# loxxous/Jampack

Measured on AMD Instinct MI355X. Metric: MB/s compress (forward BWT + rANS encode) on 64 MiB blocks; bit-exact vs CPU ref, higher is better.
Workload: dtype u8/int32; 1 GPU; enwik8-like 100000000 B per GPU as 64 MiB blocks (2 blocks), forward BWT + rANS encode, inputs resident in HBM

## Files before the change

### jampack_amd/csrc/ans_enc.hip

```cpp
#include <vector>

#include "ans_enc.hpp"
#include "chain_pool.hpp"

using namespace jpk;
using namespace jpk_enc;

namespace {

void enc_layout(Arena &a, const EncDims &d, EncBufs &b, int what, size_t sym_total = 0, size_t lane_total = 0)
{
    const size_t tiles = (size_t)d.nch * d.tpc;
    const size_t stride = d.chunk;
    const size_t nsym = sym_total ? sym_total : (size_t)d.nch * stride;
    const size_t nlane = lane_total ? lane_total : (size_t)d.nch * 4 * rans_lane_stride(stride);
    const EncBufs keep = b;
    if (what & LAY_RANK) memset(&b, 0, sizeof b); else b = keep;
    if (what & LAY_RANK) {
        b.tilecnt = a.get<uint32_t>(tiles * 256);
        b.lastpos = a.get<int32_t>(tiles * 256);
        b.freq = a.get<int32_t>((size_t)d.nch * 256);
        b.bstart = a.get<uint32_t>((size_t)d.nch * 256);
        b.ranks = a.get<uint8_t>((size_t)d.nch * stride + 64);
    }
    if (what & LAY_RLE) {
        b.lz = a.get<uint32_t>(tiles);
        b.ext = a.get<uint32_t>(tiles);
        b.tcount = a.get<uint32_t>(tiles);
        b.toff = a.get<uint32_t>(tiles);
        b.rlen = a.get<uint32_t>(d.nch + 1);
        b.rle = a.get<uint16_t>((size_t)d.nch * stride + 64);
    }
    if (what & LAY_MODEL) {
        b.dens = a.get<uint32_t>(d.nch + 64);
        b.cmap = a.get<uint32_t>(d.nch + 64);
        b.clscnt = a.get<uint32_t>(tiles * 8);
        b.clstotal = a.get<uint32_t>((size_t)d.nch * 8);
        b.ord = a.get<uint32_t>(nsym);
        b.qhist = a.get<uint32_t>((size_t)d.nch * 6 * NQ * QSTRIDE);
        b.qcdf = a.get<uint32_t>((size_t)d.nch * 6 * NQ * QSTRIDE);
        b.exph = a.get<uint16_t>(7 * nsym);
        b.mantad = a.get<uint32_t>(nsym);
        b.cls8 = a.get<uint8_t>(nsym + 64);
        b.clist = a.get<uint32_t>(2 * ((nsym + 3) & ~(size_t)3) + 64);
        const size_t segs = (size_t)d.nch * 9 * d.tpc;
        b.seg_flag = a.get<uint32_t>(segs);
        b.seg_lo = a.get<int32_t>(segs);
        b.seg_end = a.get<int32_t>(segs);
        b.seg_start = a.get<int32_t>(segs);
        b.seg_tab = a.get<uint16_t>(segs * 32);
        b.seg_miss = a.get<uint16_t>(segs);
        b.seg_reach = a.get<uint16_t>(segs);
        b.recs = a.get<uint4>(nlane + RANS_SLACK) + (a.planning ? 0 : RANS_SLACK);
        b.pairs = (what & LAY_PLAIN) ? a.get<uint32_t>((size_t)d.nch * stride * 2) : nullptr;
    }
    if (what & LAY_RANS) {
        b.x16 = a.get<uint16_t>(nlane + 64);
        b.emask = a.get<uint32_t>(nlane / 16 + 64);
        b.etsum = a.get<uint32_t>((size_t)d.nch * emit_tiles_per_chunk(stride));
        b.fstate = a.get<uint32_t>((size_t)d.nch * 4);
        b.csize = a.get<uint32_t>(d.nch);
        b.stamp = a.get<uint64_t>(2 * (size_t)d.nch);
        b.hdr = a.get<uint8_t>((size_t)d.nch * HDR_MAX);
        b.hsize = a.get<uint32_t>(d.nch);
// ... 109 lines not shown
        Arena rest(ctx, true);
        EncBufs dummy = b;
        enc_layout(rest, d, dummy, LAY_MODEL | LAY_RANS, sym_total ? sym_total : 256, lane_total ? lane_total : 512);
        if (ctx->arena_off + rest.need > ctx->arena_cap) {
            if (attempt) return JPK_E_ALLOC;
            JPK_TRY(jpk_arena_ensure(ctx, ctx->arena_off + rest.need));
            continue;
        }
        enc_layout(real, d, b, LAY_MODEL | LAY_RANS, sym_total ? sym_total : 256, lane_total ? lane_total : 512);
        d.sbase = sbase; d.lbase = lbase;
        break;
    }
    return JPK_OK;
}

int enc_launch_groups(jpk_ctx *ctx, int inflight_n, uint32_t nch)
{
    int ngroups = jpk_enc_groups_for(inflight_n, nch);
    static const long groups_env = jpk_env_long("JPK_ENC_GROUPS", 0);
    if (groups_env >= 1 && groups_env <= jpk_ctx::ENC_GROUPS && (uint32_t)groups_env <= nch) ngroups = groups_env;
    for (int g = 0; g + 1 < ngroups; g++)
        if (!ctx->aux[g] && hipStreamCreateWithFlags(&ctx->aux[g], hipStreamNonBlocking) != hipSuccess) { ctx->aux[g] = nullptr; ngroups = g + 1; break; }
    return ngroups;
}

int enc_graded_groups(jpk_ctx *ctx, const uint8_t *d_in, const EncDims &d, EncBufs &b, int ngroups)
{
    hipStream_t st = ctx->stream;
    JPK_HIP(hipMemsetAsync(b.dens, 0, (size_t)d.nch * 4, st));
    JPK_LAUNCH(ctx, PROF_ENC_HIST, d.len, k_density, dim3((d.chunk + ATILE * 4 - 1) / (ATILE * 4), d.nch), dim3(TB), d_in, d, b.dens);
    JPK_LAUNCH(ctx, PROF_ENC_HIST, 0, k_order, dim3(1), dim3(256), d, b.dens, b.cmap);
    JPK_HIP(hipEventRecord(ctx->ev_pre[0], st));
    uint32_t gsz[jpk_ctx::ENC_GROUPS];
    {
        uint32_t left = d.nch;
        for (int g = 0; g < ngroups; g++) {
            uint32_t n = (g + 1 == ngroups) ? left : d.nch >> (ngroups - g);
            if (n < 2) n = 2;
            if (n > left) n = left;
            gsz[g] = n;
            left -= n;
        }
    }
    uint32_t off = 0;
// ... 38 lines not shown
        JPK_TRY(rc);
        JPK_HIP(hipGetLastError());
        JPK_HIP(hipEventRecord(ctx->ev_done[0], lease.stream));
        JPK_HIP(hipEventSynchronize(ctx->ev_done[0]));
        lease.done();
    } else {
        JPK_TRY(run_chain(ctx, d, b));
    }
    JPK_TRY(run_emit_counts(ctx, d, b));
    return JPK_OK;
}

int encode_core(jpk_ctx *ctx, const uint8_t *d_in, EncDims &d, EncBufs &b, int inflight_n, const GroupTabs *gt = nullptr)
{
    JPK_TRY(enc_front(ctx, d_in, d, b, gt));
    JPK_HIP(hipMemsetAsync(b.qhist, 0, (size_t)d.nch * 6 * NQ * QSTRIDE * 4, ctx->stream));
    const int ngroups = enc_launch_groups(ctx, inflight_n, d.nch);
    if (ngroups >= 2) JPK_TRY(enc_graded_groups(ctx, d_in, d, b, ngroups));
    else JPK_TRY(enc_single_group(ctx, d, b));
    return run_offsets(ctx, d, b);
}
}

size_t jpk_ans_encode_arena_bytes(uint32_t len)
{
    if (len == 0) return 0;
    const EncDims d = make_dims(len, ANS_CHUNK);
    return enc_plan_bytes(d, 0, ENC_PLAN_SYM_256);
}
size_t jpk_ans_encode_arena_bytes_worst(uint32_t len)
{
// ... 130 lines not shown
}

int jpk_model_pairs_device(jpk_ctx *ctx, const uint16_t *d_rle, int32_t rlen, uint32_t *d_pairs)
{
    if (rlen == 0) return JPK_OK;
    const EncDims d = make_dims((uint32_t)rlen, (uint32_t)rlen);
    EncBufs b;
    Arena plan(ctx, true);
    enc_layout(plan, d, b, LAY_RLE | LAY_MODEL | LAY_PLAIN);
    JPK_TRY(jpk_arena_ensure(ctx, plan.need));
    Arena real(ctx, false);
    enc_layout(real, d, b, LAY_RLE | LAY_MODEL | LAY_PLAIN);
    uint32_t n = (uint32_t)rlen;
    JPK_HIP(hipMemcpyAsync(b.rlen, &n, 4, hipMemcpyHostToDevice, ctx->stream));
    JPK_HIP(hipStreamSynchronize(ctx->stream));
    JPK_HIP(hipMemsetAsync(b.qhist, 0, (size_t)d.nch * 6 * NQ * QSTRIDE * 4, ctx->stream));
    JPK_TRY(run_model(ctx, d_rle, b.rlen, d, b));
    JPK_TRY(run_pairs(ctx, d_rle, b.rlen, d, b));
    JPK_HIP(hipMemcpyAsync(d_pairs, b.pairs, (size_t)rlen * 8, hipMemcpyDeviceToDevice, ctx->stream));
    JPK_HIP(hipStreamSynchronize(ctx->stream));
    return JPK_OK;
}
```

### jampack_amd/csrc/ans_enc.hpp

```cpp
#pragma once
#include "ans_common.hpp"
#include "common.hpp"

namespace jpk_enc {
using namespace jpk;

constexpr int TB = 256;

struct EncDims {
    uint32_t len;
    uint32_t chunk;
    uint32_t nch;
    uint32_t tpc;
    uint32_t ncl;
    const uint32_t *cmap;
    const uint32_t *clen;
    const uint32_t *cblk;
    uint8_t *const *bout;
    const uint32_t *sbase;
    const uint32_t *lbase;
};
__device__ __forceinline__ uint32_t chunk_of(const EncDims &d, uint32_t i) { return d.cmap ? d.cmap[i] : i; }
__device__ __forceinline__ size_t sym_stride(const EncDims &d, uint32_t c, size_t rle_stride) { return d.sbase ? (size_t)(d.sbase[c + 1] - d.sbase[c]) : rle_stride; }
__device__ __forceinline__ size_t sym_base(const EncDims &d, uint32_t c, size_t rle_stride) { return d.sbase ? (size_t)d.sbase[c] : (size_t)c * rle_stride; }
// ... 5 lines not shown
    return left < d.chunk ? (uint32_t)left : d.chunk;
}

__host__ __device__ __forceinline__ size_t rans_lane_stride(size_t rle_stride) { return (rle_stride / 2 + 384) & ~(size_t)127; }
__device__ __forceinline__ size_t lane_stride_of(const EncDims &d, uint32_t c, size_t rle_stride) { return rans_lane_stride(sym_stride(d, c, rle_stride)); }
__device__ __forceinline__ size_t lane_base(const EncDims &d, uint32_t c, size_t rle_stride) { return d.lbase ? (size_t)d.lbase[c] : (size_t)c * 4 * rans_lane_stride(rle_stride); }

constexpr int RANS_RING = 16;
constexpr int RANS_SLACK = 16 * RANS_RING;
constexpr int ETILE = 4096;
constexpr int HDR_MAX = 259 * 5 + 1;
inline uint32_t emit_tiles_per_chunk(size_t stride) { return (uint32_t)((2 * stride + ETILE - 1) / ETILE); }

struct EncBufs {
    uint32_t *tilecnt; int32_t *lastpos; int32_t *freq; uint32_t *bstart; uint8_t *ranks;
    uint32_t *lz, *ext, *tcount, *toff, *rlen;
    uint16_t *rle;
    uint32_t *clscnt, *clstotal, *ord, *qhist, *qcdf, *dens, *cmap;
    uint8_t *cls8; uint32_t *clist;
    uint32_t *seg_flag; int32_t *seg_lo, *seg_end, *seg_start; uint16_t *seg_tab, *seg_miss, *seg_reach;
    uint16_t *exph; uint32_t *mantad, *pairs; uint4 *recs;
    uint16_t *x16; uint32_t *emask, *etsum, *fstate, *csize;
    uint64_t *stamp;
    uint8_t *hdr; uint32_t *hsize; uint64_t *outoff;
};

enum { LAY_RANK = 1, LAY_RLE = 2, LAY_MODEL = 4, LAY_RANS = 8, LAY_PLAIN = 16 };

constexpr int MAIL_TOTAL = 0;
constexpr int MAIL_RLE_SYMBOLS = 2;
constexpr int MAIL_CHAIN_CYCLES = 4;
constexpr int MAIL_CHAIN_TICKS = 6;
constexpr int MAIL_CHAIN_RLEN = 8;
constexpr int MAIL_SYM_TOTAL = 12;
constexpr int MAIL_LANE_TOTAL = 13;
// ... 20 lines not shown
```

### jampack_amd/csrc/ans_enc_front.hip

```cpp
#include "ans_enc.hpp"

using namespace jpk;
using namespace jpk_enc;

namespace {

__global__ __launch_bounds__(TB) void k_enc_hist(const uint8_t *__restrict__ in, EncDims d, uint32_t *__restrict__ tilecnt,
                                                int32_t *__restrict__ lastpos)
{
    const uint32_t c = chunk_of(d, blockIdx.y), t = blockIdx.x;
    const uint32_t clen = chunk_len(d, c), ts = t * ATILE;
    if (ts >= clen) return;
    __shared__ uint32_t h[TB / 64][256];
    __shared__ int32_t lp[TB / 64][256];
#pragma unroll
    for (int k = 0; k < TB / 64; k++) { h[k][threadIdx.x] = 0; lp[k][threadIdx.x] = -1; }
    __syncthreads();
    const uint8_t *src = in + (size_t)c * d.chunk;
    uint8_t sy[ATILE / TB];
#pragma unroll
    for (int it = 0; it < ATILE / TB; it++) {
        const uint32_t i = ts + it * TB + threadIdx.x;
        sy[it] = src[i < clen ? i : clen - 1];
    }
// ... 8 lines not shown
        if (valid && (m & lt) == 0ull) {
            h[w][s] += (uint32_t)__popcll(m);
            lp[w][s] = (int32_t)(i - (uint32_t)lane_id() + (63u - (uint32_t)__clzll((long long)m)));
        }
    }
    __syncthreads();
    size_t o = ((size_t)c * d.tpc + t) * 256 + threadIdx.x;
    uint32_t hs = 0;
    int32_t lm = -1;
#pragma unroll
    for (int k = 0; k < TB / 64; k++) { hs += h[k][threadIdx.x]; lm = lp[k][threadIdx.x] > lm ? lp[k][threadIdx.x] : lm; }
    tilecnt[o] = hs;
    lastpos[o] = lm;
}

__global__ __launch_bounds__(256) void k_enc_prep(EncDims d, uint32_t *__restrict__ tilecnt, int32_t *__restrict__ lastpos,
                                                 int32_t *__restrict__ freq, uint32_t *__restrict__ bstart)
{
    const uint32_t c = chunk_of(d, blockIdx.x), s = threadIdx.x;
    const uint32_t clen = chunk_len(d, c);
    const uint32_t nt = (clen + ATILE - 1) / ATILE;
    uint32_t f = 0;
    int32_t p = -1;
    for (uint32_t t = 0; t < nt; t++) {
        size_t o = ((size_t)c * d.tpc + t) * 256 + s;
        uint32_t n = tilecnt[o];
        tilecnt[o] = f;
        f += n;
        int32_t l = lastpos[o];
        lastpos[o] = p;
        p = l > p ? l : p;
    }
    __shared__ uint32_t sf[256];
    sf[s] = f;
    freq[(size_t)c * 256 + s] = (int32_t)f;
    __syncthreads();
    uint32_t b = 0;
    for (uint32_t k = 0; k < 256; k++) {
        uint32_t fk = sf[k];
        if (fk > f || (fk == f && k < s)) b += fk;
    }
    bstart[(size_t)c * 256 + s] = b;
}

__device__ __forceinline__ uint32_t mtf_shr1(uint32_t carry_in, uint32_t v)
{
// ... 127 lines not shown
    for (int k = 0; k < ATILE / TB; k++) {
        const uint32_t p = k * TB + threadIdx.x;
        rv[k] = src[p < tl ? p : tl - 1];
    }
#pragma unroll
    for (int k = ATILE / TB - 1; k >= 0; k--) {
        uint32_t p = k * TB + threadIdx.x;
        if (p < tl && rv[k] != 0) first = p;
    }
    __shared__ uint32_t sm[TB / 64 + 1];
    uint32_t tot;
    block_incl_scan<OpMin>(first, sm, &tot);
    if (threadIdx.x == 0) lz[(size_t)c * d.tpc + t] = tot < tl ? tot : tl;
}

__global__ void k_rle_ext(EncDims d, const uint32_t *__restrict__ lz, uint32_t *__restrict__ ext)
{
    const uint32_t ci = blockIdx.x * blockDim.x + threadIdx.x;
    if (ci >= d.ncl) return;
    const uint32_t c = chunk_of(d, ci);
    const uint32_t clen = chunk_len(d, c);
    const uint32_t nt = (clen + ATILE - 1) / ATILE;
    uint32_t e = 0;
    for (int t = (int)nt - 1; t >= 0; t--) {
        ext[(size_t)c * d.tpc + t] = e;
        uint32_t tl = (clen - t * ATILE < (uint32_t)ATILE) ? clen - t * ATILE : (uint32_t)ATILE;
        uint32_t z = lz[(size_t)c * d.tpc + t];
        e = (z == tl) ? z + e : z;
    }
}

template <bool EMIT>
__global__ __launch_bounds__(TB) void k_rle_tiles(const uint8_t *__restrict__ ranks, EncDims d, const uint32_t *__restrict__ ext,
                                                 uint32_t *__restrict__ tcount, const uint32_t *__restrict__ toff, uint16_t *__restrict__ rle,
                                                 size_t rle_stride)
{
    const uint32_t c = chunk_of(d, blockIdx.y), t = blockIdx.x;
    const uint32_t clen = chunk_len(d, c), ts = t * ATILE;
    if (ts >= clen) return;
    const uint32_t tl = (clen - ts < (uint32_t)ATILE) ? clen - ts : (uint32_t)ATILE;
    const uint8_t *src = ranks + (size_t)c * d.chunk + ts;
    const uint32_t p0 = threadIdx.x * 16;
    uint8_t v[16];
#pragma unroll
    for (int k = 0; k < 16; k++) v[k] = (p0 + k < tl) ? src[p0 + k] : (uint8_t)1;
    uint32_t first = 0xFFFFFFFFu;
#pragma unroll
    for (int k = 15; k >= 0; k--)
        if (p0 + k < tl && v[k] != 0) first = p0 + k;
    __shared__ uint32_t fz[TB];
    __shared__ uint32_t res[TB];
    __shared__ uint32_t sm[TB / 64 + 1];
    fz[threadIdx.x] = first;
    __syncthreads();
    uint32_t rv = fz[TB - 1 - threadIdx.x];
    uint32_t inc = block_incl_scan<OpMin>(rv, sm, nullptr);
    res[threadIdx.x] = inc;
    __syncthreads();
    uint32_t after = (threadIdx.x == TB - 1) ? 0xFFFFFFFFu : res[TB - 2 - threadIdx.x];
    if (after == 0xFFFFFFFFu) after = tl + ext[(size_t)c * d.tpc + t];
    uint32_t nxt[16];
    uint32_t nn = after;
#pragma unroll
    for (int k = 15; k >= 0; k--) {
        nxt[k] = nn;
        if (p0 + k < tl && v[k] != 0) nn = p0 + k;
    }
    uint32_t prev;
    if (p0 == 0) prev = (ts == 0) ? 1u : src[-1];
    else prev = (p0 - 1 < tl) ? src[p0 - 1] : 1u;
    uint32_t cnt = 0;
    uint32_t pv = prev;
#pragma unroll
    for (int k = 0; k < 16; k++) {
        if (p0 + k < tl) {
            if (v[k] != 0) cnt += 1;
            else if (pv != 0) {
                uint32_t L = nxt[k] - (p0 + k) + 1;
                cnt += 31 - __clz((int)L);
            }
            pv = v[k];
        }
    }
    uint32_t tot;
    uint32_t incl = block_incl_scan<OpSum>(cnt, sm, &tot);
    if (!EMIT) {
        if (threadIdx.x == 0) tcount[(size_t)c * d.tpc + t] = tot;
        return;
    }
    uint16_t *out = rle + (size_t)c * rle_stride + toff[(size_t)c * d.tpc + t] + (incl - cnt);
    pv = prev;
#pragma unroll
    for (int k = 0; k < 16; k++) {
        if (p0 + k < tl) {
            if (v[k] != 0) *out++ = (uint16_t)(v[k] + 1);
            else if (pv != 0) {
                uint32_t L = nxt[k] - (p0 + k) + 1;
                for (int b = 30 - __clz((int)L); b >= 0; b--) *out++ = (uint16_t)((L >> b) & 1u);
            }
            pv = v[k];
        }
    }
}

__global__ void k_tile_prefix(EncDims d, const uint32_t *__restrict__ tcount, uint32_t *__restrict__ toff, uint32_t *__restrict__ total,
                              uint32_t unit_from_len , const uint32_t *__restrict__ count_in)
{
    const uint32_t ci = blockIdx.x * blockDim.x + threadIdx.x;
    if (ci >= d.ncl) return;
    const uint32_t c = chunk_of(d, ci);
    const uint32_t n = unit_from_len ? chunk_len(d, c) : count_in[c];
    const uint32_t nt = (n + ATILE - 1) / ATILE;
    uint32_t s = 0;
    for (uint32_t t = 0; t < nt; t++) {
        uint32_t v = tcount[(size_t)c * d.tpc + t];
        toff[(size_t)c * d.tpc + t] = s;
        s += v;
    }
    total[c] = s;
}

}

namespace jpk_enc {

int run_rank(jpk_ctx *ctx, const uint8_t *d_in, const EncDims &d, EncBufs &b)
{
    JPK_LAUNCH(ctx, PROF_ENC_HIST, d.len, k_enc_hist, dim3(d.tpc, d.ncl), dim3(TB), d_in, d, b.tilecnt, b.lastpos);
    JPK_LAUNCH(ctx, PROF_ENC_HIST, d.len, k_enc_prep, dim3(d.ncl), dim3(256), d, b.tilecnt, b.lastpos, b.freq, b.bstart);
    JPK_LAUNCH(ctx, PROF_ENC_MTF, d.len, k_enc_mtf, dim3((d.tpc + 3) / 4, d.ncl), dim3(TB), d_in, d, b.tilecnt, b.lastpos, b.bstart, b.ranks);
    JPK_HIP(hipGetLastError());
    return JPK_OK;
}

int run_rle(jpk_ctx *ctx, const uint8_t *d_ranks, const EncDims &d, EncBufs &b)
{
    JPK_LAUNCH(ctx, PROF_ENC_RLE, d.len, k_rle_lz, dim3(d.tpc, d.ncl), dim3(TB), d_ranks, d, b.lz);
    JPK_LAUNCH(ctx, PROF_ENC_RLE, d.len, k_rle_ext, dim3(jpk_grid(d.ncl, 64)), dim3(64), d, b.lz, b.ext);
    JPK_LAUNCH(ctx, PROF_ENC_RLE, d.len, (k_rle_tiles<false>), dim3(d.tpc, d.ncl), dim3(TB), d_ranks, d, b.ext, b.tcount, b.toff, b.rle, (size_t)d.chunk);
    JPK_LAUNCH(ctx, PROF_ENC_RLE, d.len, k_tile_prefix, dim3(jpk_grid(d.ncl, 64)), dim3(64), d, b.tcount, b.toff, b.rlen, 1u, (const uint32_t *)nullptr);
    JPK_LAUNCH(ctx, PROF_ENC_RLE, d.len, (k_rle_tiles<true>), dim3(d.tpc, d.ncl), dim3(TB), d_ranks, d, b.ext, b.tcount, b.toff, b.rle, (size_t)d.chunk);
    JPK_HIP(hipGetLastError());
    return JPK_OK;
}

}
```

### jampack_amd/csrc/ans_enc_model.hip

```cpp
#include "ans_enc.hpp"

using namespace jpk;
using namespace jpk_enc;

namespace {

__global__ __launch_bounds__(TB) void k_cls_count(const uint16_t *__restrict__ rle, size_t rle_stride, EncDims d, const uint32_t *__restrict__ rlen,
                                                 uint32_t *__restrict__ clscnt)
{
    const uint32_t c = chunk_of(d, blockIdx.y), t = blockIdx.x;
    const uint32_t n = rlen[c], ts = t * ATILE;
    if (ts >= n) return;
    __shared__ uint32_t h[8];
    if (threadIdx.x < 8) h[threadIdx.x] = 0;
    __syncthreads();
    const uint16_t *src = rle + (size_t)c * rle_stride;
    uint32_t loc[8] = {0, 0, 0, 0, 0, 0, 0, 0};
    uint16_t sv[ATILE / TB];
#pragma unroll
    for (int it = 0; it < ATILE / TB; it++) {
        const uint32_t i = ts + it * TB + threadIdx.x;
        sv[it] = src[i < n ? i : n - 1];
    }
#pragma unroll
// ... 2 lines not shown
        if (i < n) {
            int e = sym_class(sv[it]);
#pragma unroll
            for (int k = 0; k < 8; k++) loc[k] += (e == k);
        }
    }
#pragma unroll
    for (int k = 0; k < 8; k++) {
        uint32_t s = wave_sum(loc[k]);
        if (lane_id() == 0 && s) atomicAdd(&h[k], s);
    }
    __syncthreads();
    if (threadIdx.x < 8) clscnt[((size_t)c * d.tpc + t) * 8 + threadIdx.x] = h[threadIdx.x];
}

__global__ void k_cls_prefix(EncDims d, const uint32_t *__restrict__ rlen, uint32_t *__restrict__ clscnt, uint32_t *__restrict__ clstotal)
{
    const uint32_t g = blockIdx.x * blockDim.x + threadIdx.x;
    const uint32_t k = g & 7u;
    if ((g >> 3) >= d.ncl) return;
    const uint32_t c = chunk_of(d, g >> 3);
    const uint32_t nt = (rlen[c] + ATILE - 1) / ATILE;
    uint32_t s = 0;
    for (uint32_t t = 0; t < nt; t++) {
        size_t o = ((size_t)c * d.tpc + t) * 8 + k;
        uint32_t v = clscnt[o];
        clscnt[o] = s;
        s += v;
    }
    clstotal[(size_t)c * 8 + k] = s;
}

__global__ __launch_bounds__(TB) void k_cls_ord(const uint16_t *__restrict__ rle, size_t rle_stride, EncDims d, const uint32_t *__restrict__ rlen,
                                               const uint32_t *__restrict__ clsbase, uint32_t *__restrict__ ord, uint32_t *__restrict__ qhist,
                                               uint8_t *__restrict__ cls8, uint32_t *__restrict__ clist)
{
    const uint32_t c = chunk_of(d, blockIdx.y), t = blockIdx.x;
    const uint32_t n = rlen[c], ts = t * ATILE;
    if (ts >= n) return;
    constexpr int W = TB / 64, IT = ATILE / TB;
    __shared__ uint32_t cnt[W][8];
    if (threadIdx.x < W * 8) (&cnt[0][0])[threadIdx.x] = 0;
    __syncthreads();
    const int w = threadIdx.x >> 6, l = threadIdx.x & 63;
    const uint16_t *src = rle + (size_t)c * rle_stride;
    const size_t sb = sym_base(d, c, rle_stride), cs = sym_stride(d, c, rle_stride);
    const uint64_t lt = lanemask_lt();
    uint32_t sy[IT], rk[IT];
#pragma unroll
    for (int it = 0; it < IT; it++) {
        const uint32_t i = ts + w * (64 * IT) + it * 64 + l;
        sy[it] = src[i < n ? i : n - 1];
    }
#pragma unroll
    for (int it = 0; it < IT; it++) {
        uint32_t i = ts + w * (64 * IT) + it * 64 + l;
        bool valid = i < n;
        uint32_t s = valid ? sy[it] : 0;
        sy[it] = s;
        uint32_t e = (uint32_t)sym_class(s);
        const uint64_t m = match_any<3>(e, valid);
        uint32_t below = (uint32_t)__popcll(m & lt);
        uint32_t cc = valid ? cnt[w][e] : 0;
        rk[it] = cc + below;
        if (valid && below == 0) cnt[w][e] = cc + (uint32_t)__popcll(m);
    }
    __syncthreads();
    __shared__ uint32_t lh[6][QSTRIDE];
    __shared__ int q0[8];
    for (int i = threadIdx.x; i < 6 * QSTRIDE; i += TB) (&lh[0][0])[i] = 0;
    if (threadIdx.x < 8) {
        uint32_t s = clsbase[((size_t)c * d.tpc + t) * 8 + threadIdx.x];
        q0[threadIdx.x] = qinterval(s);
#pragma unroll
        for (int k = 0; k < W; k++) { uint32_t v = cnt[k][threadIdx.x]; cnt[k][threadIdx.x] = s; s += v; }
    }
    __syncthreads();
#pragma unroll
    for (int it = 0; it < IT; it++) {
        uint32_t i = ts + w * (64 * IT) + it * 64 + l;
        if (i < n) {
            uint32_t s = sy[it];
            int e = sym_class(s);
            uint32_t k = cnt[w][e] + rk[it];
            ord[sb + i] = k;
            cls8[sb + i] = (uint8_t)(e | ((s & 1u) << 3));
            if (e < 2) clist[2 * sb + (size_t)e * ((cs + 3) & ~(size_t)3) + k] = i | ((s & 1u) << 31);
            else {
                const int q = qinterval(k);
                const uint32_t m = s - (uint32_t)class_base(e);
// ... 227 lines not shown
            }
        }
        while (t < t1) { hist[t] = (uint16_t)x; x = adapt_step(x, i, (int)(p[t] & 7u), 8); t++; }
    } else {
        ad_for_each(r, st, t0, t1, [&](uint32_t t, int m) {
            const uint32_t l0 = m ? (uint32_t)x : 0u, fr = m ? 65536u - (uint32_t)x : (uint32_t)x;
            ma[t] = l0 | (fr << 16);
            x = adapt_step(x, 1, m, 2);
        });
    }
    return x;
}

struct AdArgs {
    const uint8_t *cls8; const uint32_t *clist; size_t rle_stride; const uint32_t *rlen; const uint32_t *clstotal;
    const uint32_t *clsbase;
    uint16_t *exph; uint32_t *mantad;
    uint32_t warm;
    uint32_t *seg_flag; int32_t *seg_lo, *seg_end, *seg_start; uint16_t *seg_tab;
    uint16_t *seg_miss, *seg_reach;
};

__global__ __launch_bounds__(64) void k_adapt_a(EncDims d, AdArgs a)
{
    const uint32_t c = chunk_of(d, blockIdx.z), rec = blockIdx.y;
    const uint32_t k = blockIdx.x * 64 + threadIdx.x;
    const AdRec r(rec);
    const AdStream st = ad_stream(d, r, c, a.cls8, a.clist, a.rle_stride, a.rlen, a.clstotal);
    const uint32_t nt = (st.n + ATILE - 1) / ATILE;
    const bool valid = k < nt;
    const uint32_t t0 = valid ? k * ATILE : 0u, t1 = !valid ? 0u : (t0 + ATILE < st.n) ? t0 + ATILE : st.n;
    const uint32_t len = t1 - t0;
    const int i = r.i, A = r.A;
    int32_t lo = r.init(), hi = lo;
    if (valid && k != 0) {
        lo = r.smin(); hi = r.smax();
        ad_for_each(r, st, t0 - a.warm, t0, [&](uint32_t, int sy) { lo = adapt_step(lo, i, sy, A); hi = adapt_step(hi, i, sy, A); });
    }
    const size_t so = ((size_t)c * 9 + rec) * d.tpc + k;
    const int32_t lo0 = lo, hi0 = hi;
    const bool plat = valid && r.exp && lo != hi && hi == r.smax() && lo == r.smax() - 31;
    bool ident = false;
    if (plat) {
        const uint32_t *cb = a.clsbase + ((size_t)c * d.tpc + k) * 8;
        uint32_t reach = 0;
        for (int e = r.i; e < 8; e++) reach += ((k + 1 < nt) ? cb[8 + e] : a.clstotal[(size_t)c * 8 + e]) - cb[e];
        ident = reach == 0;
    }
    const bool walk = valid && !ident;
    bool open = walk && lo != hi, quiet = plat;
    uint32_t miss = 0, fr = 0, u = 0;
    uint16_t *hist = a.exph + 7 * sym_base(d, c, a.rle_stride) + (size_t)(rec < 7 ? rec : 0) * sym_stride(d, c, a.rle_stride);
    uint32_t *ma = a.mantad + sym_base(d, c, a.rle_stride);
    if (r.exp) {
        const uint8_t *p = st.c8 + t0;
        const int32_t top = r.smax();
        uint4 v[4];
        if (__ballot(open && 64u <= len)) {
#pragma unroll
            for (int q = 0; q < 4; q++) v[q] = *reinterpret_cast<const uint4 *>(p + ((walk && 64u <= len) ? 16 * q : 0));
        }
// ... 66 lines not shown
            for (int q = 0; q < 4; q++) v[q] = nv[q];
            u += 16;
        }
        if (walk && u > (len & ~15u)) u = len & ~15u;
    }
    if (!valid) return;
    if (ident) {
        a.seg_flag[so] = 2u;
        return;
    }
    if (open) {
        ad_for_each(r, st, t0 + u, t1, [&](uint32_t, int sy) { lo = adapt_step(lo, i, sy, A); hi = adapt_step(hi, i, sy, A); });
        a.seg_miss[so] = (uint16_t)len;
        a.seg_reach[so] = (uint16_t)fr;
        if (lo == hi) { a.seg_flag[so] = 3u; a.seg_end[so] = lo; }
        else { a.seg_flag[so] = 0u; a.seg_lo[so] = lo0; a.seg_end[so] = hi0; }
        return;
    }
    a.seg_flag[so] = miss ? 3u : 1u;
    a.seg_miss[so] = (uint16_t)miss;
    a.seg_reach[so] = (uint16_t)fr;
    a.seg_end[so] = ad_run_write(r, st, t0 + u, t1, lo, hist, ma);
}

__global__ __launch_bounds__(64) void k_adapt_tab(EncDims d, AdArgs a)
{
    const uint32_t c = chunk_of(d, blockIdx.z), rec = blockIdx.y;
    const uint32_t k = blockIdx.x * 2 + (threadIdx.x >> 5);
    const int q = threadIdx.x & 31;
    const AdRec r(rec);
    const AdStream st = ad_stream(d, r, c, a.cls8, a.clist, a.rle_stride, a.rlen, a.clstotal);
    const uint32_t nt = (st.n + ATILE - 1) / ATILE;
    if (k >= nt) return;
    const size_t so = ((size_t)c * 9 + rec) * d.tpc + k;
    if (a.seg_flag[so]) return;
    const uint32_t t0 = k * ATILE, t1 = (t0 + ATILE < st.n) ? t0 + ATILE : st.n;
    const int32_t lo = a.seg_lo[so], hi = a.seg_end[so];
    int32_t x = (lo + q < hi) ? lo + q : hi;
    const int i = r.i, A = r.A;
    ad_for_each(r, st, t0, t1, [&](uint32_t, int sy) { x = adapt_step(x, i, sy, A); });
    a.seg_tab[so * 32 + q] = (uint16_t)(x - 1);
}

__global__ __launch_bounds__(64) void k_adapt_b(EncDims d, AdArgs a)
{
    const uint32_t g = blockIdx.x * 64 + threadIdx.x;
    const uint32_t rec = g & 15u;
    if ((g >> 4) >= d.ncl || rec >= 9) return;
    const uint32_t c = chunk_of(d, g >> 4);
    const AdRec r(rec);
    const AdStream st = ad_stream(d, r, c, a.cls8, a.clist, a.rle_stride, a.rlen, a.clstotal);
    const uint32_t nt = (st.n + ATILE - 1) / ATILE;
    int32_t x = r.init();
    for (uint32_t k = 0; k < nt; k++) {
        const size_t so = ((size_t)c * 9 + rec) * d.tpc + k;
        const uint32_t flag = a.seg_flag[so];
        if (flag == 1u) x = a.seg_end[so];
        else if (flag == 2u) a.seg_start[so] = x;
        else if (flag == 3u) { a.seg_start[so] = x; x = a.seg_end[so]; }
        else {
            a.seg_start[so] = x;
            int q = x - a.seg_lo[so];
            q = q < 0 ? 0 : (q > 31 ? 31 : q);
            x = (int32_t)a.seg_tab[so * 32 + q] + 1;
        }
    }
}

__global__ __launch_bounds__(64) void k_adapt_c(EncDims d, AdArgs a)
{
    const uint32_t c = chunk_of(d, blockIdx.z), rec = blockIdx.y;
    const uint32_t k = blockIdx.x * 64 + threadIdx.x;
    const AdRec r(rec);
    const AdStream st = ad_stream(d, r, c, a.cls8, a.clist, a.rle_stride, a.rlen, a.clstotal);
    const uint32_t nt = (st.n + ATILE - 1) / ATILE;
    if (k >= nt) return;
    const size_t so = ((size_t)c * 9 + rec) * d.tpc + k;
    const uint32_t flag = a.seg_flag[so];
    if (flag == 1u) return;
    const uint32_t t0 = k * ATILE, t1 = (t0 + ATILE < st.n) ? t0 + ATILE : st.n;
    const uint32_t miss = flag == 2u ? t1 - t0 : a.seg_miss[so], fr = flag == 2u ? t1 - t0 : a.seg_reach[so];
    uint16_t *hist = a.exph + 7 * sym_base(d, c, a.rle_stride) + (size_t)(rec < 7 ? rec : 0) * sym_stride(d, c, a.rle_stride);
    const int32_t x0 = a.seg_start[so];
    if (fr) {
        const uint32_t x = (uint32_t)x0 & 0xffffu, xx = x | (x << 16);
        uint32_t t = t0;
        for (; t + 8 <= t0 + fr; t += 8) *reinterpret_cast<uint4 *>(hist + t) = make_uint4(xx, xx, xx, xx);
        for (; t < t0 + fr; t++) hist[t] = (uint16_t)x;
    }
    if (fr < miss) ad_run_write(r, st, t0 + fr, t0 + miss, x0, hist, a.mantad + sym_base(d, c, a.rle_stride));
}

}

namespace jpk_enc {

int run_model(jpk_ctx *ctx, const uint16_t *d_rle, const uint32_t *d_rlen, const EncDims &d, EncBufs &b)
{
    const size_t stride = d.chunk;
    JPK_LAUNCH(ctx, PROF_ENC_CLASS, 0, k_cls_count, dim3(d.tpc, d.ncl), dim3(TB), d_rle, stride, d, d_rlen, b.clscnt);
    JPK_LAUNCH(ctx, PROF_ENC_CLASS, 0, k_cls_prefix, dim3(jpk_grid((size_t)d.ncl * 8, 64)), dim3(64), d, d_rlen, b.clscnt, b.clstotal);
    JPK_LAUNCH(ctx, PROF_ENC_CLASS, 0, k_cls_ord, dim3(d.tpc, d.ncl), dim3(TB), d_rle, stride, d, d_rlen, b.clscnt, b.ord, b.qhist, b.cls8, b.clist);
    JPK_LAUNCH(ctx, PROF_ENC_CLASS, 0, k_quasi_build, dim3(NQ, 6, d.ncl), dim3(64), d, b.clstotal, b.qhist, b.qcdf);
    AdArgs aa;
    aa.cls8 = b.cls8; aa.clist = b.clist; aa.rle_stride = stride; aa.rlen = d_rlen; aa.clstotal = b.clstotal; aa.clsbase = b.clscnt;
    aa.exph = b.exph; aa.mantad = b.mantad;
    aa.warm = AD_WARM_DEFAULT;
    aa.seg_flag = b.seg_flag; aa.seg_lo = b.seg_lo; aa.seg_end = b.seg_end; aa.seg_start = b.seg_start; aa.seg_tab = b.seg_tab;
    aa.seg_miss = b.seg_miss; aa.seg_reach = b.seg_reach;
    JPK_LAUNCH(ctx, PROF_ENC_ADAPTIVE, 0, k_adapt_a, dim3((d.tpc + 63) / 64, 9, d.ncl), dim3(64), d, aa);
    JPK_LAUNCH(ctx, PROF_ENC_ADAPTIVE, 0, k_adapt_tab, dim3((d.tpc + 1) / 2, 9, d.ncl), dim3(64), d, aa);
    JPK_LAUNCH(ctx, PROF_ENC_ADAPTIVE, 0, k_adapt_b, dim3(jpk_grid((size_t)d.ncl * 16, 64)), dim3(64), d, aa);
    JPK_LAUNCH(ctx, PROF_ENC_ADAPTIVE, 0, k_adapt_c, dim3((d.tpc + 63) / 64, 9, d.ncl), dim3(64), d, aa);
    JPK_HIP(hipGetLastError());
    return JPK_OK;
}

}
```

Before: 6274 MB/s.

## Remove serial per-chunk prefix kernels and compact adaptive table work

New measurement: 6265 MB/s. About the same (-0.2%).

```diff
diff --git a/jampack_amd/csrc/ans_enc.hip b/jampack_amd/csrc/ans_enc.hip
--- a/jampack_amd/csrc/ans_enc.hip
+++ b/jampack_amd/csrc/ans_enc.hip
@@ -25,19 +25,19 @@
     }
     if (what & LAY_RLE) {
         b.lz = a.get<uint32_t>(tiles);
-        b.ext = a.get<uint32_t>(tiles);
         b.tcount = a.get<uint32_t>(tiles);
-        b.toff = a.get<uint32_t>(tiles);
         b.rlen = a.get<uint32_t>(d.nch + 1);
         b.rle = a.get<uint16_t>((size_t)d.nch * stride + 64);
     }
     if (what & LAY_MODEL) {
         b.dens = a.get<uint32_t>(d.nch + 64);
+        b.tab_n = a.get<uint32_t>(d.nch + 64);
+        b.qhist = a.get<uint32_t>((size_t)d.nch * 6 * NQ * QSTRIDE);
+        b.qhist_end = a.planning ? nullptr : b.qhist + (size_t)d.nch * 6 * NQ * QSTRIDE;
         b.cmap = a.get<uint32_t>(d.nch + 64);
         b.clscnt = a.get<uint32_t>(tiles * 8);
         b.clstotal = a.get<uint32_t>((size_t)d.nch * 8);
         b.ord = a.get<uint32_t>(nsym);
-        b.qhist = a.get<uint32_t>((size_t)d.nch * 6 * NQ * QSTRIDE);
         b.qcdf = a.get<uint32_t>((size_t)d.nch * 6 * NQ * QSTRIDE);
         b.exph = a.get<uint16_t>(7 * nsym);
         b.mantad = a.get<uint32_t>(nsym);
@@ -47,7 +47,7 @@
         b.seg_flag = a.get<uint32_t>(segs);
         b.seg_lo = a.get<int32_t>(segs);
         b.seg_end = a.get<int32_t>(segs);
-        b.seg_start = a.get<int32_t>(segs);
+        b.tab_list = a.get<uint32_t>(segs);
         b.seg_tab = a.get<uint16_t>(segs * 32);
         b.seg_miss = a.get<uint16_t>(segs);
         b.seg_reach = a.get<uint16_t>(segs);
@@ -187,6 +187,12 @@
     return JPK_OK;
 }
 
+int enc_clear(jpk_ctx *ctx, const EncBufs &b)
+{
+    JPK_HIP(hipMemsetAsync(b.dens, 0, (size_t)((const char *)b.qhist_end - (const char *)b.dens), ctx->stream));
+    return JPK_OK;
+}
+
 int enc_launch_groups(jpk_ctx *ctx, int inflight_n, uint32_t nch)
 {
     int ngroups = jpk_enc_groups_for(inflight_n, nch);
@@ -200,7 +206,6 @@
 int enc_graded_groups(jpk_ctx *ctx, const uint8_t *d_in, const EncDims &d, EncBufs &b, int ngroups)
 {
     hipStream_t st = ctx->stream;
-    JPK_HIP(hipMemsetAsync(b.dens, 0, (size_t)d.nch * 4, st));
     JPK_LAUNCH(ctx, PROF_ENC_HIST, d.len, k_density, dim3((d.chunk + ATILE * 4 - 1) / (ATILE * 4), d.nch), dim3(TB), d_in, d, b.dens);
     JPK_LAUNCH(ctx, PROF_ENC_HIST, 0, k_order, dim3(1), dim3(256), d, b.dens, b.cmap);
     JPK_HIP(hipEventRecord(ctx->ev_pre[0], st));
@@ -269,7 +274,7 @@
 int encode_core(jpk_ctx *ctx, const uint8_t *d_in, EncDims &d, EncBufs &b, int inflight_n, const GroupTabs *gt = nullptr)
 {
     JPK_TRY(enc_front(ctx, d_in, d, b, gt));
-    JPK_HIP(hipMemsetAsync(b.qhist, 0, (size_t)d.nch * 6 * NQ * QSTRIDE * 4, ctx->stream));
+    JPK_TRY(enc_clear(ctx, b));
     const int ngroups = enc_launch_groups(ctx, inflight_n, d.nch);
     if (ngroups >= 2) JPK_TRY(enc_graded_groups(ctx, d_in, d, b, ngroups));
     else JPK_TRY(enc_single_group(ctx, d, b));
@@ -430,7 +435,7 @@
     uint32_t n = (uint32_t)rlen;
     JPK_HIP(hipMemcpyAsync(b.rlen, &n, 4, hipMemcpyHostToDevice, ctx->stream));
     JPK_HIP(hipStreamSynchronize(ctx->stream));
-    JPK_HIP(hipMemsetAsync(b.qhist, 0, (size_t)d.nch * 6 * NQ * QSTRIDE * 4, ctx->stream));
+    JPK_TRY(enc_clear(ctx, b));
     JPK_TRY(run_model(ctx, d_rle, b.rlen, d, b));
     JPK_TRY(run_pairs(ctx, d_rle, b.rlen, d, b));
     JPK_HIP(hipMemcpyAsync(d_pairs, b.pairs, (size_t)rlen * 8, hipMemcpyDeviceToDevice, ctx->stream));
diff --git a/jampack_amd/csrc/ans_enc.hpp b/jampack_amd/csrc/ans_enc.hpp
--- a/jampack_amd/csrc/ans_enc.hpp
+++ b/jampack_amd/csrc/ans_enc.hpp
@@ -43,11 +43,13 @@
 
 struct EncBufs {
     uint32_t *tilecnt; int32_t *lastpos; int32_t *freq; uint32_t *bstart; uint8_t *ranks;
-    uint32_t *lz, *ext, *tcount, *toff, *rlen;
+    uint32_t *lz, *tcount, *rlen;
     uint16_t *rle;
     uint32_t *clscnt, *clstotal, *ord, *qhist, *qcdf, *dens, *cmap;
+    uint32_t *qhist_end;
+    uint32_t *tab_n, *tab_list;
     uint8_t *cls8; uint32_t *clist;
-    uint32_t *seg_flag; int32_t *seg_lo, *seg_end, *seg_start; uint16_t *seg_tab, *seg_miss, *seg_reach;
+    uint32_t *seg_flag; int32_t *seg_lo, *seg_end; uint16_t *seg_tab, *seg_miss, *seg_reach;
     uint16_t *exph; uint32_t *mantad, *pairs; uint4 *recs;
     uint16_t *x16; uint32_t *emask, *etsum, *fstate, *csize;
     uint64_t *stamp;
diff --git a/jampack_amd/csrc/ans_enc_front.hip b/jampack_amd/csrc/ans_enc_front.hip
--- a/jampack_amd/csrc/ans_enc_front.hip
+++ b/jampack_amd/csrc/ans_enc_front.hip
@@ -46,6 +46,8 @@
     lastpos[o] = lm;
 }
 
+constexpr int PREP_BATCH = 16;
+
 __global__ __launch_bounds__(256) void k_enc_prep(EncDims d, uint32_t *__restrict__ tilecnt, int32_t *__restrict__ lastpos,
                                                  int32_t *__restrict__ freq, uint32_t *__restrict__ bstart)
 {
@@ -54,14 +56,39 @@
     const uint32_t nt = (clen + ATILE - 1) / ATILE;
     uint32_t f = 0;
     int32_t p = -1;
-    for (uint32_t t = 0; t < nt; t++) {
-        size_t o = ((size_t)c * d.tpc + t) * 256 + s;
-        uint32_t n = tilecnt[o];
-        tilecnt[o] = f;
-        f += n;
-        int32_t l = lastpos[o];
-        lastpos[o] = p;
-        p = l > p ? l : p;
+    uint32_t *tc = tilecnt + (size_t)c * d.tpc * 256 + s;
+    int32_t *lp = lastpos + (size_t)c * d.tpc * 256 + s;
+    const uint32_t last = nt ? nt - 1 : 0;
+    uint32_t n[PREP_BATCH], nn[PREP_BATCH] = {};
+    int32_t l[PREP_BATCH], nl[PREP_BATCH] = {};
+#pragma unroll
+    for (int k = 0; k < PREP_BATCH; k++) {
+        const size_t o = (size_t)((uint32_t)k < nt ? (uint32_t)k : last) * 256;
+        n[k] = tc[o];
+        l[k] = lp[o];
+    }
+    for (uint32_t t0 = 0; t0 < nt; t0 += PREP_BATCH) {
+        if (t0 + PREP_BATCH < nt) {
+#pragma unroll
+            for (int k = 0; k < PREP_BATCH; k++) {
+                const uint32_t t = t0 + PREP_BATCH + k;
+                const size_t o = (size_t)(t < nt ? t : last) * 256;
+                nn[k] = tc[o];
+                nl[k] = lp[o];
+            }
+        }
+#pragma unroll
+        for (int k = 0; k < PREP_BATCH; k++) {
+            if (t0 + k < nt) {
+                const size_t o = (size_t)(t0 + k) * 256;
+                tc[o] = f;
+                f += n[k];
+                lp[o] = p;
+                p = l[k] > p ? l[k] : p;
+            }
+        }
+#pragma unroll
+        for (int k = 0; k < PREP_BATCH; k++) { n[k] = nn[k]; l[k] = nl[k]; }
     }
     __shared__ uint32_t sf[256];
     sf[s] = f;
@@ -219,32 +246,37 @@
     if (threadIdx.x == 0) lz[(size_t)c * d.tpc + t] = tot < tl ? tot : tl;
 }
 
-__global__ void k_rle_ext(EncDims d, const uint32_t *__restrict__ lz, uint32_t *__restrict__ ext)
-{
-    const uint32_t ci = blockIdx.x * blockDim.x + threadIdx.x;
-    if (ci >= d.ncl) return;
-    const uint32_t c = chunk_of(d, ci);
-    const uint32_t clen = chunk_len(d, c);
-    const uint32_t nt = (clen + ATILE - 1) / ATILE;
+__device__ __forceinline__ uint32_t rle_zeros_behind(const uint32_t *__restrict__ lzc, uint32_t clen, uint32_t nt, uint32_t t)
+{
+    const uint32_t l = (uint32_t)lane_id();
     uint32_t e = 0;
-    for (int t = (int)nt - 1; t >= 0; t--) {
-        ext[(size_t)c * d.tpc + t] = e;
-        uint32_t tl = (clen - t * ATILE < (uint32_t)ATILE) ? clen - t * ATILE : (uint32_t)ATILE;
-        uint32_t z = lz[(size_t)c * d.tpc + t];
-        e = (z == tl) ? z + e : z;
-    }
+    for (uint32_t u = t + 1; u < nt; u += 64) {
+        const uint32_t i = u + l;
+        const bool in = i < nt;
+        const uint32_t z = in ? lzc[i] : 0u;
+        const uint32_t tli = !in ? 0u : (clen - i * ATILE < (uint32_t)ATILE) ? clen - i * ATILE : (uint32_t)ATILE;
+        const uint64_t stop = __ballot(!in || z != tli);
+        const uint32_t upto = stop ? (uint32_t)__builtin_ctzll(stop) : 64u;
+        e += wave_sum(l <= upto ? z : 0u);
+        if (stop) break;
+    }
+    return e;
 }
 
 template <bool EMIT>
-__global__ __launch_bounds__(TB) void k_rle_tiles(const uint8_t *__restrict__ ranks, EncDims d, const uint32_t *__restrict__ ext,
-                                                 uint32_t *__restrict__ tcount, const uint32_t *__restrict__ toff, uint16_t *__restrict__ rle,
+__global__ __launch_bounds__(TB) void k_rle_tiles(const uint8_t *__restrict__ ranks, EncDims d, const uint32_t *__restrict__ lz,
+                                                 uint32_t *__restrict__ tcount, uint32_t *__restrict__ rlen, uint16_t *__restrict__ rle,
                                                  size_t rle_stride)
 {
     const uint32_t c = chunk_of(d, blockIdx.y), t = blockIdx.x;
     const uint32_t clen = chunk_len(d, c), ts = t * ATILE;
     if (ts >= clen) return;
     const uint32_t tl = (clen - ts < (uint32_t)ATILE) ? clen - ts : (uint32_t)ATILE;
+    const uint32_t nt = (clen + ATILE - 1) / ATILE;
     const uint8_t *src = ranks + (size_t)c * d.chunk + ts;
+    uint32_t before = 0;
+    if (EMIT)
+        for (uint32_t j = threadIdx.x; j < t; j += TB) before += tcount[(size_t)c * d.tpc + j];
     const uint32_t p0 = threadIdx.x * 16;
     uint8_t v[16];
 #pragma unroll
@@ -263,7 +295,8 @@
     res[threadIdx.x] = inc;
     __syncthreads();
     uint32_t after = (threadIdx.x == TB - 1) ? 0xFFFFFFFFu : res[TB - 2 - threadIdx.x];
-    if (after == 0xFFFFFFFFu) after = tl + ext[(size_t)c * d.tpc + t];
+    const uint32_t ext = (src[tl - 1] == 0 && t + 1 < nt) ? rle_zeros_behind(lz + (size_t)c * d.tpc, clen, nt, t) : 0u;
+    if (after == 0xFFFFFFFFu) after = tl + ext;
     uint32_t nxt[16];
     uint32_t nn = after;
 #pragma unroll
@@ -293,7 +326,10 @@
         if (threadIdx.x == 0) tcount[(size_t)c * d.tpc + t] = tot;
         return;
     }
-    uint16_t *out = rle + (size_t)c * rle_stride + toff[(size_t)c * d.tpc + t] + (incl - cnt);
+    uint32_t toff;
+    block_incl_scan<OpSum>(before, sm, &toff);
+    if (threadIdx.x == 0 && t + 1 == nt) rlen[c] = toff + tot;
+    uint16_t *out = rle + (size_t)c * rle_stride + toff + (incl - cnt);
     pv = prev;
 #pragma unroll
     for (int k = 0; k < 16; k++) {
@@ -308,23 +344,6 @@
     }
 }
 
-__global__ void k_tile_prefix(EncDims d, const uint32_t *__restrict__ tcount, uint32_t *__restrict__ toff, uint32_t *__restrict__ total,
-                              uint32_t unit_from_len , const uint32_t *__restrict__ count_in)
-{
-    const uint32_t ci = blockIdx.x * blockDim.x + threadIdx.x;
-    if (ci >= d.ncl) return;
-    const uint32_t c = chunk_of(d, ci);
-    const uint32_t n = unit_from_len ? chunk_len(d, c) : count_in[c];
-    const uint32_t nt = (n + ATILE - 1) / ATILE;
-    uint32_t s = 0;
-    for (uint32_t t = 0; t < nt; t++) {
-        uint32_t v = tcount[(size_t)c * d.tpc + t];
-        toff[(size_t)c * d.tpc + t] = s;
-        s += v;
-    }
-    total[c] = s;
-}
-
 }
 
 namespace jpk_enc {
@@ -341,10 +360,8 @@
 int run_rle(jpk_ctx *ctx, const uint8_t *d_ranks, const EncDims &d, EncBufs &b)
 {
     JPK_LAUNCH(ctx, PROF_ENC_RLE, d.len, k_rle_lz, dim3(d.tpc, d.ncl), dim3(TB), d_ranks, d, b.lz);
-    JPK_LAUNCH(ctx, PROF_ENC_RLE, d.len, k_rle_ext, dim3(jpk_grid(d.ncl, 64)), dim3(64), d, b.lz, b.ext);
-    JPK_LAUNCH(ctx, PROF_ENC_RLE, d.len, (k_rle_tiles<false>), dim3(d.tpc, d.ncl), dim3(TB), d_ranks, d, b.ext, b.tcount, b.toff, b.rle, (size_t)d.chunk);
-    JPK_LAUNCH(ctx, PROF_ENC_RLE, d.len, k_tile_prefix, dim3(jpk_grid(d.ncl, 64)), dim3(64), d, b.tcount, b.toff, b.rlen, 1u, (const uint32_t *)nullptr);
-    JPK_LAUNCH(ctx, PROF_ENC_RLE, d.len, (k_rle_tiles<true>), dim3(d.tpc, d.ncl), dim3(TB), d_ranks, d, b.ext, b.tcount, b.toff, b.rle, (size_t)d.chunk);
+    JPK_LAUNCH(ctx, PROF_ENC_RLE, d.len, (k_rle_tiles<false>), dim3(d.tpc, d.ncl), dim3(TB), d_ranks, d, b.lz, b.tcount, b.rlen, b.rle, (size_t)d.chunk);
+    JPK_LAUNCH(ctx, PROF_ENC_RLE, d.len, (k_rle_tiles<true>), dim3(d.tpc, d.ncl), dim3(TB), d_ranks, d, b.lz, b.tcount, b.rlen, b.rle, (size_t)d.chunk);
     JPK_HIP(hipGetLastError());
     return JPK_OK;
 }
diff --git a/jampack_amd/csrc/ans_enc_model.hip b/jampack_amd/csrc/ans_enc_model.hip
--- a/jampack_amd/csrc/ans_enc_model.hip
+++ b/jampack_amd/csrc/ans_enc_model.hip
@@ -40,34 +40,21 @@
     if (threadIdx.x < 8) clscnt[((size_t)c * d.tpc + t) * 8 + threadIdx.x] = h[threadIdx.x];
 }
 
-__global__ void k_cls_prefix(EncDims d, const uint32_t *__restrict__ rlen, uint32_t *__restrict__ clscnt, uint32_t *__restrict__ clstotal)
-{
-    const uint32_t g = blockIdx.x * blockDim.x + threadIdx.x;
-    const uint32_t k = g & 7u;
-    if ((g >> 3) >= d.ncl) return;
-    const uint32_t c = chunk_of(d, g >> 3);
-    const uint32_t nt = (rlen[c] + ATILE - 1) / ATILE;
-    uint32_t s = 0;
-    for (uint32_t t = 0; t < nt; t++) {
-        size_t o = ((size_t)c * d.tpc + t) * 8 + k;
-        uint32_t v = clscnt[o];
-        clscnt[o] = s;
-        s += v;
-    }
-    clstotal[(size_t)c * 8 + k] = s;
-}
-
 __global__ __launch_bounds__(TB) void k_cls_ord(const uint16_t *__restrict__ rle, size_t rle_stride, EncDims d, const uint32_t *__restrict__ rlen,
-                                               const uint32_t *__restrict__ clsbase, uint32_t *__restrict__ ord, uint32_t *__restrict__ qhist,
-                                               uint8_t *__restrict__ cls8, uint32_t *__restrict__ clist)
+                                               const uint32_t *__restrict__ clscnt, uint32_t *__restrict__ clstotal, uint32_t *__restrict__ ord,
+                                               uint32_t *__restrict__ qhist, uint8_t *__restrict__ cls8, uint32_t *__restrict__ clist)
 {
     const uint32_t c = chunk_of(d, blockIdx.y), t = blockIdx.x;
     const uint32_t n = rlen[c], ts = t * ATILE;
     if (ts >= n) return;
     constexpr int W = TB / 64, IT = ATILE / TB;
     __shared__ uint32_t cnt[W][8];
+    __shared__ uint32_t cbase[8];
     if (threadIdx.x < W * 8) (&cnt[0][0])[threadIdx.x] = 0;
+    if (threadIdx.x < 8) cbase[threadIdx.x] = 0;
     __syncthreads();
+    uint32_t front = 0;
+    for (uint32_t j = threadIdx.x >> 3; j < t; j += TB / 8) front += clscnt[((size_t)c * d.tpc + j) * 8 + (threadIdx.x & 7u)];
     const int w = threadIdx.x >> 6, l = threadIdx.x & 63;
     const uint16_t *src = rle + (size_t)c * rle_stride;
     const size_t sb = sym_base(d, c, rle_stride), cs = sym_stride(d, c, rle_stride);
@@ -91,15 +78,20 @@
         rk[it] = cc + below;
         if (valid && below == 0) cnt[w][e] = cc + (uint32_t)__popcll(m);
     }
+    front += __shfl_xor(front, 8, 64);
+    front += __shfl_xor(front, 16, 64);
+    front += __shfl_xor(front, 32, 64);
+    if (l < 8 && front) atomicAdd(&cbase[l], front);
     __syncthreads();
     __shared__ uint32_t lh[6][QSTRIDE];
     __shared__ int q0[8];
     for (int i = threadIdx.x; i < 6 * QSTRIDE; i += TB) (&lh[0][0])[i] = 0;
     if (threadIdx.x < 8) {
-        uint32_t s = clsbase[((size_t)c * d.tpc + t) * 8 + threadIdx.x];
+        uint32_t s = cbase[threadIdx.x];
         q0[threadIdx.x] = qinterval(s);
 #pragma unroll
         for (int k = 0; k < W; k++) { uint32_t v = cnt[k][threadIdx.x]; cnt[k][threadIdx.x] = s; s += v; }
+        if (ts + ATILE >= n) clstotal[(size_t)c * 8 + threadIdx.x] = s;
     }
     __syncthreads();
 #pragma unroll
@@ -357,10 +349,11 @@
 
 struct AdArgs {
     const uint8_t *cls8; const uint32_t *clist; size_t rle_stride; const uint32_t *rlen; const uint32_t *clstotal;
-    const uint32_t *clsbase;
+    const uint32_t *clscnt;
     uint16_t *exph; uint32_t *mantad;
     uint32_t warm;
-    uint32_t *seg_flag; int32_t *seg_lo, *seg_end, *seg_start; uint16_t *seg_tab;
+    uint32_t *seg_flag; int32_t *seg_lo, *seg_end; uint16_t *seg_tab;
+    uint32_t *tab_n, *tab_list;
     uint16_t *seg_miss, *seg_reach;
 };
 
@@ -385,9 +378,9 @@
     const bool plat = valid && r.exp && lo != hi && hi == r.smax() && lo == r.smax() - 31;
     bool ident = false;
     if (plat) {
-        const uint32_t *cb = a.clsbase + ((size_t)c * d.tpc + k) * 8;
+        const uint32_t *cn = a.clscnt + ((size_t)c * d.tpc + k) * 8;
         uint32_t reach = 0;
-        for (int e = r.i; e < 8; e++) reach += ((k + 1 < nt) ? cb[8 + e] : a.clstotal[(size_t)c * 8 + e]) - cb[e];
+        for (int e = r.i; e < 8; e++) reach += cn[e];
         ident = reach == 0;
     }
     const bool walk = valid && !ident;
@@ -484,7 +477,10 @@
         a.seg_miss[so] = (uint16_t)len;
         a.seg_reach[so] = (uint16_t)fr;
         if (lo == hi) { a.seg_flag[so] = 3u; a.seg_end[so] = lo; }
-        else { a.seg_flag[so] = 0u; a.seg_lo[so] = lo0; a.seg_end[so] = hi0; }
+        else {
+            a.seg_flag[so] = 0u; a.seg_lo[so] = lo0; a.seg_end[so] = hi0;
+            a.tab_list[atomicAdd(a.tab_n, 1u)] = (uint32_t)so;
+        }
         return;
     }
     a.seg_flag[so] = miss ? 3u : 1u;
@@ -493,48 +489,53 @@
     a.seg_end[so] = ad_run_write(r, st, t0 + u, t1, lo, hist, ma);
 }
 
+constexpr uint32_t AD_TAB_GRID = 256;
 __global__ __launch_bounds__(64) void k_adapt_tab(EncDims d, AdArgs a)
 {
-    const uint32_t c = chunk_of(d, blockIdx.z), rec = blockIdx.y;
-    const uint32_t k = blockIdx.x * 2 + (threadIdx.x >> 5);
+    const uint32_t n = *a.tab_n;
     const int q = threadIdx.x & 31;
-    const AdRec r(rec);
-    const AdStream st = ad_stream(d, r, c, a.cls8, a.clist, a.rle_stride, a.rlen, a.clstotal);
-    const uint32_t nt = (st.n + ATILE - 1) / ATILE;
-    if (k >= nt) return;
-    const size_t so = ((size_t)c * 9 + rec) * d.tpc + k;
-    if (a.seg_flag[so]) return;
-    const uint32_t t0 = k * ATILE, t1 = (t0 + ATILE < st.n) ? t0 + ATILE : st.n;
-    const int32_t lo = a.seg_lo[so], hi = a.seg_end[so];
-    int32_t x = (lo + q < hi) ? lo + q : hi;
-    const int i = r.i, A = r.A;
-    ad_for_each(r, st, t0, t1, [&](uint32_t, int sy) { x = adapt_step(x, i, sy, A); });
-    a.seg_tab[so * 32 + q] = (uint16_t)(x - 1);
-}
-
-__global__ __launch_bounds__(64) void k_adapt_b(EncDims d, AdArgs a)
-{
-    const uint32_t g = blockIdx.x * 64 + threadIdx.x;
-    const uint32_t rec = g & 15u;
-    if ((g >> 4) >= d.ncl || rec >= 9) return;
-    const uint32_t c = chunk_of(d, g >> 4);
-    const AdRec r(rec);
-    const AdStream st = ad_stream(d, r, c, a.cls8, a.clist, a.rle_stride, a.rlen, a.clstotal);
-    const uint32_t nt = (st.n + ATILE - 1) / ATILE;
-    int32_t x = r.init();
-    for (uint32_t k = 0; k < nt; k++) {
-        const size_t so = ((size_t)c * 9 + rec) * d.tpc + k;
-        const uint32_t flag = a.seg_flag[so];
-        if (flag == 1u) x = a.seg_end[so];
-        else if (flag == 2u) a.seg_start[so] = x;
-        else if (flag == 3u) { a.seg_start[so] = x; x = a.seg_end[so]; }
-        else {
-            a.seg_start[so] = x;
-            int q = x - a.seg_lo[so];
+    for (uint32_t li = blockIdx.x * 2 + (threadIdx.x >> 5); li < n; li += gridDim.x * 2) {
+        const size_t so = a.tab_list[li];
+        const uint32_t k = (uint32_t)(so % d.tpc), cr = (uint32_t)(so / d.tpc), rec = cr % 9u, c = cr / 9u;
+        const AdRec r(rec);
+        const AdStream st = ad_stream(d, r, c, a.cls8, a.clist, a.rle_stride, a.rlen, a.clstotal);
+        const uint32_t t0 = k * ATILE, t1 = (t0 + ATILE < st.n) ? t0 + ATILE : st.n;
+        const int32_t lo = a.seg_lo[so], hi = a.seg_end[so];
+        int32_t x = (lo + q < hi) ? lo + q : hi;
+        const int i = r.i, A = r.A;
+        ad_for_each(r, st, t0, t1, [&](uint32_t, int sy) { x = adapt_step(x, i, sy, A); });
+        a.seg_tab[so * 32 + q] = (uint16_t)(x - 1);
+    }
+}
+
+constexpr int AD_BACK = 8;
+__device__ __forceinline__ int32_t ad_start_state(const AdRec &r, const AdArgs &a, size_t so0, uint32_t k)
+{
+    int32_t j = (int32_t)k - 1, cst = -1;
+    bool tables = false;
+    while (j >= 0 && cst < 0) {
+        uint32_t f[AD_BACK];
+#pragma unroll
+        for (int q = 0; q < AD_BACK; q++) f[q] = a.seg_flag[so0 + (uint32_t)(j - q > 0 ? j - q : 0)];
+#pragma unroll
+        for (int q = 0; q < AD_BACK; q++) {
+            if (cst < 0 && j - q >= 0) {
+                if (f[q] & 1u) cst = j - q;
+                else if (f[q] == 0u) tables = true;
+            }
+        }
+        j -= AD_BACK;
+    }
+    int32_t x = cst < 0 ? r.init() : a.seg_end[so0 + (uint32_t)cst];
+    if (tables) {
+        for (uint32_t m = (uint32_t)(cst + 1); m < k; m++) {
+            if (a.seg_flag[so0 + m] != 0u) continue;
+            int q = x - a.seg_lo[so0 + m];
             q = q < 0 ? 0 : (q > 31 ? 31 : q);
-            x = (int32_t)a.seg_tab[so * 32 + q] + 1;
-        }
-    }
+            x = (int32_t)a.seg_tab[(so0 + m) * 32 + q] + 1;
+        }
+    }
+    return x;
 }
 
 __global__ __launch_bounds__(64) void k_adapt_c(EncDims d, AdArgs a)
@@ -545,13 +546,13 @@
     const AdStream st = ad_stream(d, r, c, a.cls8, a.clist, a.rle_stride, a.rlen, a.clstotal);
     const uint32_t nt = (st.n + ATILE - 1) / ATILE;
     if (k >= nt) return;
-    const size_t so = ((size_t)c * 9 + rec) * d.tpc + k;
+    const size_t so0 = ((size_t)c * 9 + rec) * d.tpc, so = so0 + k;
     const uint32_t flag = a.seg_flag[so];
     if (flag == 1u) return;
     const uint32_t t0 = k * ATILE, t1 = (t0 + ATILE < st.n) ? t0 + ATILE : st.n;
     const uint32_t miss = flag == 2u ? t1 - t0 : a.seg_miss[so], fr = flag == 2u ? t1 - t0 : a.seg_reach[so];
     uint16_t *hist = a.exph + 7 * sym_base(d, c, a.rle_stride) + (size_t)(rec < 7 ? rec : 0) * sym_stride(d, c, a.rle_stride);
-    const int32_t x0 = a.seg_start[so];
+    const int32_t x0 = ad_start_state(r, a, so0, k);
     if (fr) {
         const uint32_t x = (uint32_t)x0 & 0xffffu, xx = x | (x << 16);
         uint32_t t = t0;
@@ -569,18 +570,18 @@
 {
     const size_t stride = d.chunk;
     JPK_LAUNCH(ctx, PROF_ENC_CLASS, 0, k_cls_count, dim3(d.tpc, d.ncl), dim3(TB), d_rle, stride, d, d_rlen, b.clscnt);
-    JPK_LAUNCH(ctx, PROF_ENC_CLASS, 0, k_cls_prefix, dim3(jpk_grid((size_t)d.ncl * 8, 64)), dim3(64), d, d_rlen, b.clscnt, b.clstotal);
-    JPK_LAUNCH(ctx, PROF_ENC_CLASS, 0, k_cls_ord, dim3(d.tpc, d.ncl), dim3(TB), d_rle, stride, d, d_rlen, b.clscnt, b.ord, b.qhist, b.cls8, b.clist);
+    JPK_LAUNCH(ctx, PROF_ENC_CLASS, 0, k_cls_ord, dim3(d.tpc, d.ncl), dim3(TB), d_rle, stride, d, d_rlen, b.clscnt, b.clstotal, b.ord, b.qhist, b.cls8, b.clist);
     JPK_LAUNCH(ctx, PROF_ENC_CLASS, 0, k_quasi_build, dim3(NQ, 6, d.ncl), dim3(64), d, b.clstotal, b.qhist, b.qcdf);
     AdArgs aa;
-    aa.cls8 = b.cls8; aa.clist = b.clist; aa.rle_stride = stride; aa.rlen = d_rlen; aa.clstotal = b.clstotal; aa.clsbase = b.clscnt;
+    aa.cls8 = b.cls8; aa.clist = b.clist; aa.rle_stride = stride; aa.rlen = d_rlen; aa.clstotal = b.clstotal; aa.clscnt = b.clscnt;
     aa.exph = b.exph; aa.mantad = b.mantad;
     aa.warm = AD_WARM_DEFAULT;
-    aa.seg_flag = b.seg_flag; aa.seg_lo = b.seg_lo; aa.seg_end = b.seg_end; aa.seg_start = b.seg_start; aa.seg_tab = b.seg_tab;
+    aa.seg_flag = b.seg_flag; aa.seg_lo = b.seg_lo; aa.seg_end = b.seg_end; aa.seg_tab = b.seg_tab;
     aa.seg_miss = b.seg_miss; aa.seg_reach = b.seg_reach;
+    const size_t first = d.cmap ? (size_t)(d.cmap - b.cmap) : 0;
+    aa.tab_n = b.tab_n + first; aa.tab_list = b.tab_list + first * 9 * d.tpc;
     JPK_LAUNCH(ctx, PROF_ENC_ADAPTIVE, 0, k_adapt_a, dim3((d.tpc + 63) / 64, 9, d.ncl), dim3(64), d, aa);
-    JPK_LAUNCH(ctx, PROF_ENC_ADAPTIVE, 0, k_adapt_tab, dim3((d.tpc + 1) / 2, 9, d.ncl), dim3(64), d, aa);
-    JPK_LAUNCH(ctx, PROF_ENC_ADAPTIVE, 0, k_adapt_b, dim3(jpk_grid((size_t)d.ncl * 16, 64)), dim3(64), d, aa);
+    JPK_LAUNCH(ctx, PROF_ENC_ADAPTIVE, 0, k_adapt_tab, dim3(AD_TAB_GRID), dim3(64), d, aa);
     JPK_LAUNCH(ctx, PROF_ENC_ADAPTIVE, 0, k_adapt_c, dim3((d.tpc + 63) / 64, 9, d.ncl), dim3(64), d, aa);
     JPK_HIP(hipGetLastError());
     return JPK_OK;
```
